# NSAPH-Projects/weather2alert

Hardware: AMD Instinct MI355X
Metric: env_steps_per_sec (higher is better)
Workload: dtype f32 tables, fp64 logit accumulation, f32 sigmoid/reward

## Files before the change

### include/w2a.h

```cpp
#ifndef W2A_H
#define W2A_H

#include <stddef.h>
#include <stdint.h>

#ifdef __cplusplus
extern "C" {
#endif

#define W2A_ABI_VERSION 18
#define W2A_ROW_FLOATS 32

enum {
  W2A_OK = 0,
  W2A_ERR_ARG = -1,
  W2A_ERR_SCHEMA = -2,
  W2A_ERR_HIP = -3,
  W2A_ERR_STATE = -4
};

enum {
  W2A_ST_BAD_EPISODE = 1,
  W2A_ST_BAD_ACTION = 2,
  W2A_ST_STEP_AFTER_DONE = 4,
  W2A_ST_STALE_GRAPH = 8
};

enum { W2A_ACT_I32 = 0, W2A_ACT_I64 = 1, W2A_ACT_U8 = 2 };

enum {
  W2A_STEP_AUTORESET = 1,
  W2A_STEP_NO_OBS = 2,
  W2A_STEP_CLASSIC = 8,
  W2A_STEP_WIDE = 32,
  W2A_STEP_UNPACKED = 128,
  W2A_STEP_NEXT_STEP = 256,
  W2A_STEP_NO_CAPTURE = 512,
  W2A_STEP_SKIP_FINISHED = 64,
  W2A_STEP_REWARD_GIVEN = 16
};

enum { W2A_BUDGET_FIXED = 0, W2A_BUDGET_LESS_THAN = 1, W2A_BUDGET_CENTERED = 2 };

typedef struct w2a_tables {
  const float *X;
  const int32_t *n_days;
  const int32_t *B0;
  const float *W;
  const int32_t *fips_to_weather;
  const int32_t *sim_cnt;
  int32_t T, S_w, Y, S, n_samples;
  int32_t n_obs;
  int32_t obs_slot[W2A_ROW_FLOATS];
  int32_t slot_heat_qi;
  const int32_t *sim_ptr;
  const int32_t *sim_idx;
  int32_t slot_alerts_2wks;
  const uint32_t *gate_bits;
  int32_t gate_words;
} w2a_tables;

typedef struct w2a_env w2a_env;

typedef struct w2a_state_view {
  int32_t *t, *used, *streak, *hist14, *last_actual, *at_budget, *budget, *n_days;
  int32_t *county_w, *year_i, *coef_col, *sample, *sticky_budget, *episode_no;
  int32_t *finished;
  float *episode_return;
} w2a_state_view;

int w2a_abi_version(void);
const char *w2a_last_error(void);

size_t w2a_state_bytes(int64_t num_envs);

int w2a_create(const w2a_tables *tables, int64_t num_envs, int64_t env_gid0, void *state, size_t state_bytes,
               int32_t *status, w2a_env **out);
void w2a_destroy(w2a_env *env);

int w2a_reset(w2a_env *env, const int32_t *county_w, const int32_t *year_i, const int32_t *coef_col,
              const int32_t *sample, const int32_t *budget, const uint8_t *mask, float *obs, void *stream);

int w2a_reset_device_rng(w2a_env *env, uint64_t seed, int32_t location, int augment, int32_t budget_kw,
                         int sample_budget_mode, int sticky, int restart_episodes, const uint8_t *mask, float *obs,
                         void *stream);

int w2a_set_autoreset(w2a_env *env, uint64_t seed, int32_t location, int augment, int32_t budget_kw,
                      int sample_budget_mode, int sticky);

int w2a_step(w2a_env *env, const void *actions, int action_dtype, float *obs, float *reward, uint8_t *done,
// ... 332 lines not shown
```

### weather2alert_amd/_ffi.py

```python
from __future__ import annotations

import ctypes as C
import os

from . import build as _build

ROW_FLOATS = 32

OK = 0
ST_BAD_EPISODE, ST_BAD_ACTION, ST_STEP_AFTER_DONE, ST_STALE_GRAPH = 1, 2, 4, 8
ACT_I32, ACT_I64, ACT_U8 = 0, 1, 2
STEP_AUTORESET, STEP_NO_OBS, STEP_CLASSIC, STEP_REWARD_GIVEN, STEP_WIDE, STEP_SKIP_FINISHED, STEP_UNPACKED, STEP_NEXT_STEP, STEP_NO_CAPTURE = 1, 2, 8, 16, 32, 64, 128, 256, 512
S64_MIN_ENVS = 131072
ABI_VERSION = 18
FIX_BITS = {"alert_2wks": 1, "lag": 2, "penalty": 4, "obs": 8, "augment": 16}
BUDGET_FIXED, BUDGET_LESS_THAN, BUDGET_CENTERED = 0, 1, 2

SYMBOLS = [
    "w2a_abi_version", "w2a_last_error", "w2a_state_bytes", "w2a_create", "w2a_destroy", "w2a_reset",
    "w2a_reset_device_rng", "w2a_set_autoreset", "w2a_step", "w2a_get_state", "w2a_read_status",
    "w2a_sort_workspace_bytes", "w2a_sort_episodes", "w2a_reset_device_rng_sorted", "w2a_observe", "w2a_rollout", "w2a_rollout_order_workspace_bytes", "w2a_rollout_order_attach", "w2a_rollout_order", "w2a_rollout_posterior_mean", "w2a_policy_actions", "w2a_set_semantics",
    "w2a_group_workspace_bytes", "w2a_group_by_column", "w2a_posterior_mean_reward", "w2a_set_posterior_kernel", "w2a_set_episode_word", "w2a_invalidate", "w2a_query", "w2a_rollout_mfma_workspace_bytes", "w2a_rollout_mfma_prepare",
    "w2a_rollout_linear", "w2a_rollout_mlp", "w2a_rollout_linear_record", "w2a_rollout_mlp_record",
    "w2a_posterior_returns", "w2a_hindsight_workspace_bytes", "w2a_hindsight_optimum",
    "w2a_policy_gradient_workspace_bytes", "w2a_policy_gradient_linear",
    "w2a_policy_gradient_mlp_workspace_bytes", "w2a_policy_gradient_mlp",
    "w2a_imitation_gradient_linear", "w2a_imitation_gradient_mlp_workspace_bytes", "w2a_imitation_gradient_mlp",
    "w2a_imitation_gradient_linear_weighted", "w2a_imitation_gradient_mlp_weighted",
    "w2a_value_gradient_linear_workspace_bytes", "w2a_value_gradient_linear",
    "w2a_value_gradient_mlp_workspace_bytes", "w2a_value_gradient_mlp",
    "w2a_value_gradient_linear_gae_workspace_bytes", "w2a_value_gradient_linear_gae",
    "w2a_value_gradient_mlp_gae_workspace_bytes", "w2a_value_gradient_mlp_gae",
    "w2a_surrogate_gradient_linear", "w2a_surrogate_gradient_mlp_workspace_bytes", "w2a_surrogate_gradient_mlp",
    "w2a_alert_gate", "w2a_rollout_linear_gated", "w2a_policy_gradient_linear_gated",
    "w2a_imitation_gradient_linear_gated", "w2a_surrogate_gradient_linear_gated", "w2a_hindsight_optimum_gated",
    "w2a_rollout_mlp_gated", "w2a_policy_gradient_mlp_gated", "w2a_imitation_gradient_mlp_gated",
    "w2a_surrogate_gradient_mlp_gated",
    "w2a_fisher_vector_product_linear", "w2a_fisher_vector_product_mlp_workspace_bytes",
    "w2a_fisher_vector_product_mlp",
    "w2a_q_gradient_mlp_workspace_bytes", "w2a_q_gradient_mlp",
    "w2a_actor_critic_mlp_workspace_bytes", "w2a_actor_critic_mlp",
    "w2a_lookahead_rollout_linear", "w2a_lookahead_rollout_linear_gated", "w2a_lookahead_rollout_mlp",
    "w2a_lookahead_rollout_mlp_gated", "w2a_lookahead_policy_gradient_linear",
    "w2a_lookahead_imitation_gradient_linear",
    "w2a_hindsight_along", "w2a_relabel_imitation_linear", "w2a_relabel_imitation_mlp",
    "w2a_hindsight_curve_workspace_bytes", "w2a_hindsight_curve", "w2a_hindsight_curve_gated",
]
Q_LOCKSTEP_DAY, Q_PACKED_ELIGIBLE, Q_PACKED_CURRENT, Q_CANONICAL_CURRENT, Q_LAST_ROLLOUT_KERNEL, Q_LAST_STEP_KERNEL, Q_LOCKSTEP = 0, 1, 2, 3, 4, 5, 6
Q_EPISODE_WORD_BYTES = 7
ROLLOUT_KERNELS = {0: "k_rollout", 1: "k_rollout64", 2: "k_rollout_mfma", 3: "k_rollout_linear", 4: "k_rollout_mlp"}
PM_KERNELS = {"vector": 0, "matrix": 1, "matrix_i8": 2}
POLICY_KINDS = {"never": 0, "always": 1, "bernoulli": 2, "threshold": 3, "table": 4}


class Policy(C.Structure):
    _fields_ = [("kind", C.c_int32), ("p", C.c_float), ("obs_col", C.c_int32), ("threshold", C.c_float),
                ("obs_lag", C.c_int32), ("require_budget", C.c_int32), ("table", C.c_void_p),
                ("table_R", C.c_int32), ("seed", C.c_uint64)]


class LinearPolicy(C.Structure):
    _fields_ = [("weight", C.c_void_p), ("bias", C.c_void_p), ("group", C.c_void_p), ("n_groups", C.c_int32),
                ("sample", C.c_int32), ("require_budget", C.c_int32), ("seed", C.c_uint64)]


# ... 264 lines not shown
```

### weather2alert_amd/csrc/w2a_bookkeeping.h

```cpp
#ifndef W2A_BOOKKEEPING_H
#define W2A_BOOKKEEPING_H

#include <stdint.h>

struct W2aBook {
  int pk_valid, canon_valid;
  int pk_static_ok;
  int lock;
  int32_t uni_t;
  int32_t uni_nd;
  int graph_canon;
  int graph_packed;
  int graph_autoreset;
  int poisoned;
  int perm_valid;
  int has_order;
  int rm_valid;
  int has_order_ws;
  int hist_valid;
  int last_step_kernel, last_rollout_kernel;
};

enum { W2A_BK_STEP_CLASSIC = 0, W2A_BK_STEP_WIDE = 1, W2A_BK_STEP_PACKED = 2 };
enum { W2A_BK_ROLLOUT_4LANE = 0, W2A_BK_ROLLOUT_WIDE = 1, W2A_BK_ROLLOUT_MFMA = 2 };
// ... 59 lines not shown
  const bool unpacked = (masked || observe_only) && !before.canon_valid;
  b = before;
  if (unpacked) b.canon_valid = 1;
  b.hist_valid = 0; b.perm_valid = 0; b.rm_valid = 0;
}

struct BkStepPlan {
  int kernel;
  int32_t uni_nd;
  int converted;
};
template <class Dev>
static inline BkStepPlan bk_step(W2aBook &b, Dev &d, bool wide_wanted, bool autoreset, bool given, bool unpacked_flag,
                                 bool capturing) {
  BkStepPlan p;
  p.kernel = W2A_BK_STEP_CLASSIC; p.uni_nd = b.uni_nd; p.converted = 0;
  bool packed = wide_wanted && !given && !unpacked_flag && bk_can_pack(b);
  if (capturing) {
    if (packed && !b.pk_valid) packed = false;
    if (!packed && !b.canon_valid) { p.kernel = -1; return p; }
  }
  if (autoreset) {
    b.perm_valid = 0;
    b.rm_valid = 0;
    b.hist_valid = 0;
  }
  if (capturing) {
    if (packed) b.graph_packed = 1;
    else b.graph_canon = 1;
    if (autoreset) b.graph_autoreset = 1;
  }
  int32_t uni_next = (!autoreset && b.uni_t >= 0 && b.uni_t + 1 < b.uni_nd) ? b.uni_t + 1 : -1;
  if (bk_any_graph(b)) uni_next = -1;
  if (packed) {
    if (!b.pk_valid) {
      d.pack_state();
      b.pk_valid = 1; b.poisoned = 0;
      p.converted = 1;
    }
    p.kernel = W2A_BK_STEP_PACKED;
    b.canon_valid = 0;
    b.uni_t = uni_next;
    b.last_step_kernel = W2A_BK_STEP_PACKED;
    return p;
  }
  if (wide_wanted) p.kernel = W2A_BK_STEP_WIDE;
  if (!b.canon_valid) p.converted = 2;
  bk_ensure_canonical(b, d);
  bk_canonical_modified(b, true);
  b.uni_t = uni_next;
  b.last_step_kernel = p.kernel;
  return p;
}
static inline void bk_step_rollback(W2aBook &b, const W2aBook &before, const BkStepPlan &p) {
  const W2aBook after = b;
  b = before;
  b.graph_canon = after.graph_canon; b.graph_packed = after.graph_packed; b.graph_autoreset = after.graph_autoreset;
  if (bk_any_graph(b)) b.uni_t = -1;
  if (p.converted == 1) { b.pk_valid = 1; b.poisoned = 0; }
  if (p.converted == 2) b.canon_valid = 1;
}

template <class Dev>
static inline bool bk_rollout_begin(W2aBook &b, Dev &d, int32_t n_steps) {
  const int32_t day = b.uni_t;
  bk_ensure_canonical(b, d);
  bk_canonical_modified(b, true);
  b.uni_t = (day >= 0 && day + n_steps < b.uni_nd && !bk_any_graph(b)) ? day + n_steps : -1;
  return b.lock != 0;
}
static inline int bk_rollout_kernel(W2aBook &b, bool lock, bool fixes, bool mfma_built, bool wide_built) {
  int k = (wide_built && b.has_order) ? W2A_BK_ROLLOUT_WIDE : W2A_BK_ROLLOUT_4LANE;
  if (b.rm_valid && b.has_order && !fixes && lock && mfma_built) k = W2A_BK_ROLLOUT_MFMA;
  b.last_rollout_kernel = k;
  return k;
}

template <class Dev>
static inline void bk_sort(W2aBook &b, Dev &d) {
  bk_ensure_canonical(b, d);
  bk_canonical_modified(b, true);
  b.rm_valid = 0;
  b.perm_valid = 0;
  b.hist_valid = 0;
}
static inline void bk_grouped(W2aBook &b) { b.perm_valid = b.graph_autoreset ? 0 : 1; }
static inline void bk_order_attach(W2aBook &b, bool drops_order = false) {
  b.has_order_ws = 1; b.hist_valid = 0;
  if (drops_order) { b.has_order = 0; b.rm_valid = 0; }
}
static inline void bk_order_set(W2aBook &b) { b.has_order = 1; b.rm_valid = 0; }
static inline void bk_rm_prepared(W2aBook &b) { b.rm_valid = b.graph_autoreset ? 0 : 1; }

static inline void bk_invalidate(W2aBook &b) {
  b.pk_valid = 0; b.canon_valid = 1; b.lock = 0; b.uni_t = -1; b.perm_valid = 0;
  b.rm_valid = 0;
  b.hist_valid = 0;
  b.poisoned = 0;
}

#endif
```

### weather2alert_amd/csrc/w2a_step64.hip.h

```cpp
#ifndef W2A_STEP64_HIP_H
#define W2A_STEP64_HIP_H

#ifndef W2A_S64_MIN_ENVS
#define W2A_S64_MIN_ENVS 131072
#endif
#define S64_ENVS 64
#define S64_WAVES (BLOCK / 64)
#define S64_PASS_ENVS 32
#define S64_ROUNDS 4
#define S64_LIST_ROUNDS 4

struct Day {
  uint32_t t, used, streak, hist, ndays, atb, actual, used2, hist2, st_bits, last;
  int32_t budget, act;
  bool done;
};
__device__ __forceinline__ Day derive_day(const u3 h, const u3 c, int32_t act) {
  Day d;
  d.st_bits = 0;
  if (act != 0 && act != 1) { d.st_bits |= W2A_ST_BAD_ACTION; act = 1; }
  d.act = act;
  d.last = D0_LAST(h.a);
  d.t = D0_T(h.a); d.used = D0_USED(h.a); d.streak = D0_STREAK(h.a);
  d.hist = D1_HIST(h.b); d.ndays = D1_NDAYS(h.b);
// ... 63 lines not shown
#ifndef W2A_S64_SERPENTINE
#define W2A_S64_SERPENTINE 1
#endif
__device__ __forceinline__ uint32_t logical_block_rev(uint32_t b, uint32_t per_xcd) {
#if W2A_XCD_SWIZZLE
  return (b & 7u) * per_xcd + (per_xcd - 1u - (b >> 3));
#else
  return 8u * per_xcd - 1u - b;
#endif
}
template <bool WRITE_OBS, bool REWARD_GIVEN, bool AUTORESET, bool FIXES>
__host__ __device__ constexpr int s64_issue_rounds() {
  return (!WRITE_OBS || (FIXES && !AUTORESET)) ? S64_ROUNDS : 2 * S64_ROUNDS;
}
template <bool WRITE_OBS, bool REWARD_GIVEN, bool PACKED, bool AUTORESET = false, bool FIXES = false, bool NARROW = false>
__device__ __forceinline__ void s64_tile(const StepArgs &a, S64WaveT<FIXES> &sw, const int lane, const int64_t wave_env0,
                                         const bool valid, const uint32_t e, const u3 h, const u3 c, const int32_t act,
                                         const int4 so) {
  const Day d = derive_day(h, c, act);
  const uint32_t t = d.t, used2 = d.used2, hist2 = d.hist2, streak = d.streak, ndays = d.ndays;
  const uint32_t actual = d.actual, atb = d.atb, st_bits = d.st_bits;
  const int32_t budget = d.budget;
  const bool done = d.done;
  const bool restart_in = AUTORESET && a.next_step && D1_FIN(h.b);
  const uint32_t pk0 = NARROW ? pk_rem8(budget - (int32_t)used2) : used2;
  if (NARROW && (uint32_t)budget >= PK_REM_ESCAPE && valid && !restart_in && !(a.skip_finished && D1_FIN(h.b)))
    pk_rem_of(a.st, a.n)[e] = (uint32_t)(budget - (int32_t)used2);
  const uint32_t fx = FIXES ? a.tb.fixes : 0u;
  const bool fix_obs = FIXES && WRITE_OBS && (fx & W2A_FIX_OBS);
  uint32_t need_eff = actual;
  if (a.tb.gate_bits && actual)
    need_eff = (a.tb.gate_bits[t * (uint32_t)a.tb.gate_words + (c.b >> 5)] >> (c.b & 31u)) & 1u;
  const unsigned long long eff_mask = REWARD_GIVEN ? 0ull : __ballot(need_eff != 0u);
  const int n_eff = __popcll(eff_mask);
  if (!REWARD_GIVEN && need_eff)
    sw.elist[__builtin_amdgcn_mbcnt_hi((uint32_t)(eff_mask >> 32), __builtin_amdgcn_mbcnt_lo((uint32_t)eff_mask, 0u))] = (uint8_t)lane;
  {
    const uint32_t day_row = t * (uint32_t)(a.tb.S_w * a.tb.Y) + c.b;
    const uint32_t wrow = NARROW ? c.c : W_COL(c.c) * (uint32_t)a.tb.n_samples + W_SAMPLE(c.c);
    sw.desc[lane] = make_uint2((day_row * (ROWF / 4)) | ((fix_obs && !done) ? 0x80000000u : 0u),
                               (wrow * (2 * ROWF / 4)) | (need_eff << 31));
    sw.rt[lane] = runtime_fields(d, (fx & W2A_FIX_LAG) != 0u);
    if (fix_obs)
      sw.rt2[FIXES ? lane : 0] = make_float4((float)actual, (float)(actual ? streak + 1 : 0), (float)(budget - (int32_t)used2),
                                 (float)__popc(hist2));
  }
  __builtin_amdgcn_fence(__ATOMIC_RELEASE, "wavefront");
  __builtin_amdgcn_wave_barrier();
  __builtin_amdgcn_fence(__ATOMIC_ACQUIRE, "wavefront");

  const int p = lane & 7;
  const int g = lane >> 3;
  const int n_obs = a.tb.n_obs;
  const bool write_me = valid && (!done || fix_obs) && !restart_in;
  const uint32_t next_day = (uint32_t)(a.tb.S_w * a.tb.Y) * (ROWF / 4);
  constexpr int NI = s64_issue_rounds<WRITE_OBS, REWARD_GIVEN, AUTORESET, FIXES>();
  auto eff_issue = [&](const int idx, float4 &xe, float4 &we, int &je) {
    const bool has = idx < n_eff;
    je = has ? (int)sw.elist[idx & (S64_ENVS - 1)] : g;
    const uint2 ds = sw.desc[je];
    xe = a.tb.X[(ds.x & 0x7FFFFFFFu) + p];
    we = a.tb.W[(ds.y & 0x7FFFFFFFu) + (has ? ROWF / 4 : 0) + p];
  };
  auto eff_logit = [&](const int idx, float4 xe, const float4 we, const int je) {
    if (p == RT_QUAD) xe = sw.rt[je];
    if (FIXES && (fx & W2A_FIX_ALERTS_2WKS) && a.tb.slot_hist2w >= 0 && p == (a.tb.slot_hist2w >> 2))
      set_comp4(xe, a.tb.slot_hist2w & 3, sw.rt[je].w);
    double ze = (double)xe.x * (double)we.x;
    ze = fma((double)xe.y, (double)we.y, ze);
    ze = fma((double)xe.z, (double)we.z, ze);
    ze = fma((double)xe.w, (double)we.w, ze);
    if (p == GATE_QUAD && !(xe.z > 0.5f)) ze = -__builtin_inf();
    ze += dpp_f64<0xB1>(ze);
    ze += dpp_f64<0x4E>(ze);
    ze += dpp_f64<0x141>(ze);
    if (p == 0 && idx < n_eff) sw.z[je].y = (float)ze;
  };
  float4 lx0 = make_float4(0.f, 0.f, 0.f, 0.f), lw0 = lx0;
  int lj0 = 0;
  if (!REWARD_GIVEN && NI < 2 * S64_ROUNDS) eff_issue(g, lx0, lw0, lj0);
#pragma unroll 1
  for (int r0 = 0; r0 < S64_ENVS / 8; r0 += NI) {
    if (REWARD_GIVEN && !WRITE_OBS) break;
    if (wave_env0 + r0 * 8 >= a.n) break;
    float4 x[NI], wb[NI], xo[FIXES ? NI : 1];
    bool nxt[NI];
#pragma unroll
    for (int r = 0; r < NI; ++r) {
      uint2 ds = sw.desc[(r0 + r) * 8 + g];
      nxt[r] = FIXES && (ds.x >> 31) != 0u;
      if (FIXES) ds.x &= 0x7FFFFFFFu;
      x[r] = a.tb.X[ds.x + p];
      if (fix_obs) xo[r] = a.tb.X[ds.x + (nxt[r] ? next_day : 0u) + p];
      wb[r] = make_float4(0.f, 0.f, 0.f, 0.f);
      if (!REWARD_GIVEN) wb[r] = a.tb.W[(ds.y & 0x7FFFFFFFu) + p];
      if (!REWARD_GIVEN && NI == 2 * S64_ROUNDS && r == S64_ROUNDS - 1) eff_issue(g, lx0, lw0, lj0);
    }
#if W2A_S64_PRIO
    __builtin_amdgcn_s_setprio(W2A_S64_PRIO);
#endif
#pragma unroll
    for (int r = 0; r < NI; ++r) {
      const int j = (r0 + r) * 8 + g;
      if (p == RT_QUAD) x[r] = sw.rt[j];
      if (FIXES && (fx & W2A_FIX_ALERTS_2WKS) && a.tb.slot_hist2w >= 0) {
        const float a2w = sw.rt[j].w;
        if (p == (a.tb.slot_hist2w >> 2)) set_comp4(x[r], a.tb.slot_hist2w & 3, a2w);
// ... 102 lines not shown
    const float eff = need_eff ? sigmoid_f32(z.y) : 0.0f;
    r = -(1000.0f / 152.0f) * base * (1.0f - eff);
    if (FIXES && (fx & W2A_FIX_PENALTY) && d.act == 1 && atb) r = -1.0f;
  }
  const uint32_t t2 = done ? t : t + 1;
  const uint32_t streak2 = done ? streak : (actual ? streak + 1 : 0);
  const float ret = __uint_as_float(h.c) + r;
  u3 h2;
  h2.a = pack_d0(t2, used2, streak2, actual, atb);
  h2.b = pack_d1(hist2, ndays, done ? 1u : 0u);
  h2.c = __float_as_uint(ret);
#if W2A_S64_SC1 & 2
  if (PACKED) st8_sc1(&a.st.pk_hot[e], v2u{pk_pack_hot(pk0, streak2, hist2, done ? 1u : 0u), h2.c});
  else st12_sc1(&a.st.hot3[e], v3u{h2.a, h2.b, h2.c});
  if (!REWARD_GIVEN) st4_sc1(&a.reward[e], __float_as_uint(r));
  st1_sc1(&a.done[e], done ? 1u : 0u);
#else
  if (PACKED) a.st.pk_hot[e] = make_uint2(pk_pack_hot(pk0, streak2, hist2, done ? 1u : 0u), h2.c);
  else a.st.hot3[e] = h2;
  if (!REWARD_GIVEN) a.reward[e] = r;
  a.done[e] = done ? 1 : 0;
#endif
  if (PACKED && lane == 0) a.st.pk_day[wave_env0 >> 6] = t2;
  if (done && a.last_return) a.last_return[e] = ret;
  if (st_bits) atomicOr(a.status, (int)st_bits);
  }
  if (AUTORESET) {
    const bool rs = valid && (a.next_step ? restart_in : done);
    const unsigned long long rs_mask = __ballot(rs);
    if (rs_mask) {
      uint2 ds = make_uint2(0xFFFFFFFFu, 0u);
      if (rs) {
        const uint4 cold = load_cold(a.st, e);
        const Episode ep = draw_episode(a.tb, a.rc, (uint64_t)(a.gid0 + e), cold.w + 1, (int32_t)cold.z);
        if (ep.bad) atomicOr(a.status, (int)W2A_ST_BAD_EPISODE);
        store_episode(a.st, e, make_uint4(ep.ep_row, ep.ep_w, (uint32_t)ep.sticky, cold.w + 1),
                      make_uint4(pack_d0(0, 0, 0, 0, 0), pack_d1(0, ep.ndays, 0), __float_as_uint(0.0f), (uint32_t)ep.budget));
        if (PACKED && NARROW) {
          a.st.pk_hot[e] = make_uint2(pk_pack_hot(pk_rem8(ep.budget), 0u, 0u, 0u), __float_as_uint(0.0f));
          reinterpret_cast<uint32_t *>(a.st.pk_c)[e] = pk_narrow_word(ep.ep_row, ep.ep_w, (uint32_t)a.tb.n_samples, a.pk_kw);
          pk_rem_of(a.st, a.n)[e] = (uint32_t)ep.budget;
        } else if (PACKED) {
          a.st.pk_hot[e] = make_uint2(pk_pack_hot(0u, 0u, 0u, 0u), __float_as_uint(0.0f));
          a.st.pk_c[e] = make_uint2(pk_budget16((uint32_t)ep.budget) | (W_COL(ep.ep_w) << 16),
                                    (ep.ep_row & 0x3FFFFFu) | (W_SAMPLE(ep.ep_w) << 22));
        }
        ds = make_uint2(ep.ep_row * (ROWF / 4), (uint32_t)ep.budget);
      }
      if (WRITE_OBS) {
        sw.desc[lane] = ds;
        __builtin_amdgcn_fence(__ATOMIC_RELEASE, "wavefront");
        __builtin_amdgcn_wave_barrier();
        __builtin_amdgcn_fence(__ATOMIC_ACQUIRE, "wavefront");
#pragma unroll 1
        for (int r = 0; r < S64_ENVS / 8; ++r) {
          if (!((rs_mask >> (r * 8)) & 0xFFull)) continue;
          const int j = r * 8 + g;
          const uint2 dj = sw.desc[j];
          if (dj.x != 0xFFFFFFFFu) {
            float4 v = a.tb.X[dj.x + p];
            if (p == RT_QUAD) v = make_float4(0.0f, 0.0f, (float)(int32_t)dj.y, 0.0f);
            if (FIXES && (fx & W2A_FIX_ALERTS_2WKS) && a.tb.slot_hist2w >= 0 && p == (a.tb.slot_hist2w >> 2))
              set_comp4(v, a.tb.slot_hist2w & 3, 0.0f);
            float *row = reinterpret_cast<float *>(a.obs) + (size_t)(wave_env0 + j) * n_obs;
            if (so.x >= 0) row[so.x] = v.x;
            if (so.y >= 0) row[so.y] = v.y;
            if (so.z >= 0) row[so.z] = v.z;
            if (so.w >= 0) row[so.w] = v.w;
          }
        }
      }
      if (PACKED && lane == 0) a.st.pk_day[wave_env0 >> 6] = 0u;
    }
  }
}

template <bool NARROW>
__device__ __forceinline__ void s64_load_packed(const StepArgs &a, uint32_t e, uint32_t day, u3 &h, u3 &c, int32_t &act) {
  if (NARROW) {
    const uint32_t *ew = reinterpret_cast<const uint32_t *>(a.st.pk_c);
#if W2A_S64_NT_STATE & 4
    const v2u phv = __builtin_nontemporal_load(reinterpret_cast<const v2u *>(&a.st.pk_hot[e]));
    const uint2 ph = make_uint2(phv.x, phv.y);
    const uint32_t w = __builtin_nontemporal_load(&ew[e]);
#else
    const uint2 ph = a.st.pk_hot[e];
    const uint32_t w = ew[e];
#endif
    const uint32_t used = 0u;
    c.a = PK_USED(ph.x);
    if (c.a == PK_REM_ESCAPE) c.a = pk_rem_of(a.st, a.n)[e];
    h.a = pack_d0(day, used, PK_STREAK(ph.x), PK_HIST(ph.x) & 1u, 0u);
    h.b = pack_d1(PK_HIST(ph.x), (uint32_t)a.uni_nd, PK_FIN(ph.x));
    h.c = ph.y;
    c.b = w >> a.pk_kw;
    c.c = w & ((1u << a.pk_kw) - 1u);
    act = load_action(a, e);
    return;
  }
#if W2A_S64_NT_STATE & 4
  const v2u phv = __builtin_nontemporal_load(reinterpret_cast<const v2u *>(&a.st.pk_hot[e]));
  const v2u pcv = __builtin_nontemporal_load(reinterpret_cast<const v2u *>(&a.st.pk_c[e]));
  const uint2 ph = make_uint2(phv.x, phv.y), pc = make_uint2(pcv.x, pcv.y);
#else
  const uint2 ph = a.st.pk_hot[e];
  const uint2 pc = a.st.pk_c[e];
#endif
  h.a = pack_d0(day, PK_USED(ph.x), PK_STREAK(ph.x), PK_HIST(ph.x) & 1u, 0u);
  h.b = pack_d1(PK_HIST(ph.x), (uint32_t)a.uni_nd, PK_FIN(ph.x));
  h.c = ph.y;
  c.a = pc.x & 0xFFFFu;
  if (c.a == PK_BUDGET_ESCAPE) c.a = a.st.stepc[e].a;
  c.b = pc.y & 0x3FFFFFu;
  c.c = PACK_W(pc.x >> 16, pc.y >> 22);
  act = load_action(a, e);
}
__device__ __forceinline__ void s64_load_state(const StepArgs &a, uint32_t e, u3 &h, u3 &c, int32_t &act) {
#if W2A_S64_NT_STATE & 1
  const v3u hv = __builtin_nontemporal_load(reinterpret_cast<const v3u *>(&a.st.hot3[e]));
  h.a = hv.x; h.b = hv.y; h.c = hv.z;
#else
// ... 106 lines not shown
```

### weather2alert_amd/csrc/w2a_step_dispatch.hip.h

```cpp
#ifndef W2A_STEP_DISPATCH_HIP_H
#define W2A_STEP_DISPATCH_HIP_H

int w2a_step(w2a_env *env, const void *actions, int action_dtype, float *obs, float *reward, uint8_t *done,
             float *last_return, int flags, void *stream) {
  if (!env || !actions || !reward || !done) return fail(W2A_ERR_ARG, "w2a_step: NULL argument");
  if (action_dtype < W2A_ACT_I32 || action_dtype > W2A_ACT_U8) return fail(W2A_ERR_ARG, "w2a_step: bad action_dtype");
  const bool no_obs = (flags & W2A_STEP_NO_OBS) != 0;
  const bool autoreset = (flags & W2A_STEP_AUTORESET) != 0;
  const bool given = (flags & W2A_STEP_REWARD_GIVEN) != 0;
  if (given && (autoreset || env->tb.fixes || (flags & W2A_STEP_CLASSIC)))
    return fail(W2A_ERR_ARG, "w2a_step: W2A_STEP_REWARD_GIVEN is served by the 64-envs-per-wave kernel only (no in-kernel "
                             "autoreset, no corrected-semantics flags)");
  if (!no_obs && !obs) return fail(W2A_ERR_ARG, "w2a_step: obs is NULL (pass W2A_STEP_NO_OBS for reward-only)");
  if (!no_obs && ((uintptr_t)obs & 15)) return fail(W2A_ERR_ARG, "w2a_step: obs must be 16-B aligned");
  if (autoreset && !env->has_autoreset) return fail(W2A_ERR_ARG, "w2a_step: W2A_STEP_AUTORESET needs w2a_set_autoreset first");
  StepArgs a;
  memset(&a, 0, sizeof(a));
  a.tb = env->tb; a.slot_obs = env->slot_obs; a.st = env->st;
  a.actions = actions; a.obs = obs; a.reward = reward; a.done = done; a.last_return = last_return;
  a.status = env->status; a.n = env->n; a.gid0 = env->gid0; a.rc = env->autoreset; a.act_dtype = action_dtype;
  a.skip_finished = (flags & W2A_STEP_SKIP_FINISHED) ? 1 : 0;
  a.next_step = (flags & W2A_STEP_NEXT_STEP) ? 1 : 0;
  if (a.next_step && !autoreset) return fail(W2A_ERR_ARG, "w2a_step: W2A_STEP_NEXT_STEP goes with W2A_STEP_AUTORESET");
  if (a.skip_finished && !given)
    return fail(W2A_ERR_ARG, "w2a_step: W2A_STEP_SKIP_FINISHED goes with W2A_STEP_REWARD_GIVEN (policy loops)");
  dim3 grid(grid_for(env->n)), block(BLOCK);
  hipStream_t s = (hipStream_t)stream;
  const bool capturing = stream_is_capturing(s);
  if (capturing && (flags & W2A_STEP_NO_CAPTURE))
    return fail(W2A_ERR_STATE, "w2a_step: the stream is recording a hipGraph, but this loop's episode boundaries are driven "
                               "from the host (W2A_STEP_NO_CAPTURE): a reset between two steps cannot be recorded. Let the "
                               "step kernel restart finished envs itself (W2A_STEP_AUTORESET; HeatAlertVecEnv(lockstep=False))");
  const bool wide = (given || (flags & W2A_STEP_WIDE) || env->n >= W2A_S64_MIN_ENVS) && !(flags & W2A_STEP_CLASSIC);
  HipDev dv{env, s};
  const W2aBook before = env->bk;
  const BkStepPlan plan = bk_step(env->bk, dv, wide, autoreset, given, (flags & W2A_STEP_UNPACKED) != 0, capturing);
  if (plan.kernel < 0)
    return fail(W2A_ERR_STATE, "w2a_step: this step runs on the canonical state words, which are not current (the state is "
                               "in its packed lock-step form), and a conversion cannot be recorded into a hipGraph; call "
                               "w2a_get_state before capturing -- or, on a handle with a recorded packed step, do not "
                               "record a step of another kind");
#define W2A_STEP_TRY(expr) \
  do { hipError_t _e = (expr); \
       if (_e != hipSuccess) { bk_step_rollback(env->bk, before, plan); if (!capturing) bk_end_call(env->bk, dv); \
                               return fail(W2A_ERR_HIP, #expr ": %s", hipGetErrorString(_e)); } } while (0)
  if (plan.kernel != W2A_BK_STEP_CLASSIC) {
    const int64_t per_wg = (int64_t)BLOCK * W2A_S64_TILES;
    const int64_t tiles = (env->n + per_wg - 1) / per_wg;
    dim3 grid64((unsigned)(((tiles + 7) / 8) * 8));
    a.walk_rev = env->s64_launches++ & 1u;
    a.pk_kw = -1;
    if (plan.kernel == W2A_BK_STEP_PACKED) {
      a.uni_nd = plan.uni_nd;
      a.pk_kw = env->ew.narrow ? env->ew.kw : -1;
#define W2A_LAUNCH_PK(NW)                                                                                                \
      do {                                                                                                               \
        if (autoreset) {   \
          if (env->tb.fixes) {                                                                                           \
            if (no_obs) hipLaunchKernelGGL((k_step64<false, false, true, true, true, NW>), grid64, block, 0, s, a);      \
            else hipLaunchKernelGGL((k_step64<true, false, true, true, true, NW>), grid64, block, 0, s, a);              \
          } else if (no_obs) hipLaunchKernelGGL((k_step64<false, false, true, true, false, NW>), grid64, block, 0, s, a); \
          else hipLaunchKernelGGL((k_step64<true, false, true, true, false, NW>), grid64, block, 0, s, a);               \
        } else if (env->tb.fixes) {   \
          if (no_obs) hipLaunchKernelGGL((k_step64<false, false, true, false, true, NW>), grid64, block, 0, s, a);       \
          else hipLaunchKernelGGL((k_step64<true, false, true, false, true, NW>), grid64, block, 0, s, a);               \
        } else if (no_obs) hipLaunchKernelGGL((k_step64<false, false, true, false, false, NW>), grid64, block, 0, s, a); \
        else hipLaunchKernelGGL((k_step64<true, false, true, false, false, NW>), grid64, block, 0, s, a);                \
      } while (0)
      if (env->ew.narrow) W2A_LAUNCH_PK(true);
      else W2A_LAUNCH_PK(false);
#undef W2A_LAUNCH_PK
      W2A_STEP_TRY(hipGetLastError());
      bk_end_call(env->bk, dv);
      return W2A_OK;
    }
    if (given) {
      if (no_obs) hipLaunchKernelGGL((k_step64<false, true>), grid64, block, 0, s, a);
      else hipLaunchKernelGGL((k_step64<true, true>), grid64, block, 0, s, a);
    } else if (env->tb.fixes) {
      if (autoreset) {
        if (no_obs) hipLaunchKernelGGL((k_step64<false, false, false, true, true>), grid64, block, 0, s, a);
        else hipLaunchKernelGGL((k_step64<true, false, false, true, true>), grid64, block, 0, s, a);
      } else {
        if (no_obs) hipLaunchKernelGGL((k_step64<false, false, false, false, true>), grid64, block, 0, s, a);
        else hipLaunchKernelGGL((k_step64<true, false, false, false, true>), grid64, block, 0, s, a);
      }
    } else if (autoreset) {
      if (no_obs) hipLaunchKernelGGL((k_step64<false, false, false, true>), grid64, block, 0, s, a);
      else hipLaunchKernelGGL((k_step64<true, false, false, true>), grid64, block, 0, s, a);
    } else {
      if (no_obs) hipLaunchKernelGGL((k_step64<false, false>), grid64, block, 0, s, a);
      else hipLaunchKernelGGL((k_step64<true, false>), grid64, block, 0, s, a);
    }
    W2A_STEP_TRY(hipGetLastError());
    if (!capturing) bk_end_call(env->bk, dv);
    return W2A_OK;
  }
#define W2A_LAUNCH(AR, OB) \
  do { if (env->tb.fixes) hipLaunchKernelGGL((k_step<AR, OB, true>), grid, block, 0, s, a); \
       else hipLaunchKernelGGL((k_step<AR, OB, false>), grid, block, 0, s, a); } while (0)
  if (autoreset) { if (no_obs) W2A_LAUNCH(true, false); else W2A_LAUNCH(true, true); }
  else { if (no_obs) W2A_LAUNCH(false, false); else W2A_LAUNCH(false, true); }
#undef W2A_LAUNCH
  W2A_STEP_TRY(hipGetLastError());
#undef W2A_STEP_TRY
  if (!capturing) bk_end_call(env->bk, dv);
  return W2A_OK;
}

#endif
```

### weather2alert_amd/env.py

```python
from __future__ import annotations

import ctypes as C
from typing import Literal

import numpy as np
import torch

from . import _ffi, policy as _policy, stats as _stats
from .info import _LazyInfo
from .options import KernelOptions
from .rng import numpy_parity_episode
from .spaces import Box, Discrete
from .tables import CompiledTables, DeviceTables, compile_from_files

_ACT_CODES = {torch.int32: _ffi.ACT_I32, torch.int64: _ffi.ACT_I64, torch.uint8: _ffi.ACT_U8,
              torch.bool: _ffi.ACT_U8}
_BUDGET_MODES = {"less_than": _ffi.BUDGET_LESS_THAN, "centered": _ffi.BUDGET_CENTERED}
_cur_device = getattr(torch._C, "_cuda_getDevice", torch.cuda.current_device)

try:
    from gymnasium.vector import VectorEnv as _VectorEnvBase
except ImportError:
    _VectorEnvBase = object
try:
# ... 159 lines not shown
                self._group_ws = torch.empty(self._lib.w2a_group_workspace_bytes(n, ct.S, ct.n_samples), dtype=torch.uint8,
                                             device=dev)
        nd = np.unique(ct.n_days)
        uniform = len(nd) == 1 and nd[0] > 0
        if episode_order == "sorted":
            if not uniform:
                raise ValueError("episode_order='sorted' needs one episode length for every (county, year)")
            if lockstep is False:
                raise ValueError("episode_order='sorted' implies lockstep")
            with torch.cuda.device(dev):
                self._sort_ws = torch.empty(self._lib.w2a_sort_workspace_bytes(n), dtype=torch.uint8, device=dev)
        if lockstep and not uniform:
            raise ValueError("lockstep=True needs one episode length for every (county, year)")
        self._episode_len = int(nd[0]) if uniform else 0
        self._lockstep = bool(uniform and self.seed_mode == "device" and lockstep is not False)
        self._steps_in_episode = 0
        self._pending_reset = False
        self._reset_cfg = None
        self._set_step_mode()
        self._w2a_step = self._lib.w2a_step
        self._raw_stream = getattr(torch._C, "_cuda_getCurrentRawStream", None)
        self._sticky = [budget] * n
        self._needs_reset = True
        self._obs_current = False
        self._last_opts: dict = {}
        self._np_random = None
        self._np_random_seed = None

    @property
    def unwrapped(self):
        return self

    @property
    def np_random(self) -> np.random.Generator:
        if self._np_random is None:
            self._np_random_seed = int(np.random.SeedSequence().entropy % (2**63))
            self._np_random = np.random.default_rng(self._np_random_seed)
        return self._np_random

    @np_random.setter
    def np_random(self, value: np.random.Generator):
        self._np_random, self._np_random_seed = value, -1

    @property
    def np_random_seed(self):
        self.np_random
        return self._np_random_seed

    def _set_step_mode(self):
        auto = self.autoreset in ("same_step", "next_step") and self.seed_mode == "device"
        self._dev_auto = auto and not self._lockstep
        self._host_auto = auto and self._lockstep and self.autoreset == "same_step"
        self._host_next = auto and self._lockstep and self.autoreset == "next_step"
        if not self._host_next:
            self._pending_reset = False
        if self.reward_mode == "posterior_mean" and self._dev_auto:
            raise ValueError("reward_mode='posterior_mean' cannot run with the in-kernel autoreset (batches that left "
                             "lock step); use autoreset='disabled' or whole-batch resets")
        self._pm = self.reward_mode == "posterior_mean"
        host_driven = self._host_auto or self._host_next or (self.autoreset == "same_step" and not self._dev_auto)
        self._step_flags = ((0 if self.write_obs else _ffi.STEP_NO_OBS) |
                            (_ffi.STEP_NO_CAPTURE if host_driven else 0) |
                            (_ffi.STEP_REWARD_GIVEN if self._pm else 0) |
                            (_ffi.STEP_CLASSIC if self.step_kernel == "classic" else 0) |
                            (_ffi.STEP_WIDE if self.step_kernel in ("wide", "wide_unpacked") else 0) |
                            (_ffi.STEP_UNPACKED if self.step_kernel in ("unpacked", "wide_unpacked") else 0) |
                            (_ffi.STEP_AUTORESET if self._dev_auto else 0) |
                            (_ffi.STEP_NEXT_STEP if self._dev_auto and self.autoreset == "next_step" else 0))

    @property
    def step_kernel_name(self) -> str:
        wide = self._pm or self.step_kernel in ("wide", "wide_unpacked") or (self.step_kernel in ("auto", "unpacked") and
                                                          self.num_envs >= _ffi.S64_MIN_ENVS)
        return "k_step64" if (wide and self.step_kernel != "classic") else "k_step"

    @property
    def last_step_kernel(self) -> str | None:
        return {0: "k_step", 1: "k_step64", 2: "k_step64<packed>"}.get(
            self._lib.w2a_query(self._h, _ffi.Q_LAST_STEP_KERNEL))

    @property
    def packed_state(self) -> bool:
        return bool(self._lib.w2a_query(self._h, _ffi.Q_PACKED_CURRENT)) and not bool(
            self._lib.w2a_query(self._h, _ffi.Q_CANONICAL_CURRENT))

    @property
    def episode_word_bytes(self) -> int:
        return int(self._lib.w2a_query(self._h, _ffi.Q_EPISODE_WORD_BYTES))

    @property
    def last_rollout_kernel(self) -> str | None:
        return _ffi.ROLLOUT_KERNELS.get(self._lib.w2a_query(self._h, _ffi.Q_LAST_ROLLOUT_KERNEL))

    def _stream(self):
        if self._raw_stream is not None:
            return self._raw_stream(self._dev_index)
        return torch.cuda.current_stream(self.device).cuda_stream

    def close(self, **kwargs):
        if getattr(self, "_h", None):
            torch.cuda.synchronize(self.device)
            self._lib.w2a_destroy(self._h)
            self._h = None
        self._look_tables = {}
        self.closed = True

# ... 269 lines not shown
            if self.pm_kernel_choice is None:
                self._pick_pm_kernel()

    def _pick_pm_kernel(self, reps: int = 3):
        act = torch.zeros(self.num_envs, dtype=torch.int32, device=self.device)
        best = {}
        with torch.cuda.device(self.device):
            for name, code in _ffi.PM_KERNELS.items():
                _ffi.check(self._lib.w2a_set_posterior_kernel(self._h, code), "w2a_set_posterior_kernel")
                times = []
                for _ in range(reps + 1):
                    e0, e1 = torch.cuda.Event(enable_timing=True), torch.cuda.Event(enable_timing=True)
                    e0.record()
                    _ffi.check(self._lib.w2a_posterior_mean_reward(self._h, act.data_ptr(), _ffi.ACT_I32, self._rew_ptr,
                                                                   self._stream()), "w2a_posterior_mean_reward")
                    e1.record()
                    e1.synchronize()
                    times.append(e0.elapsed_time(e1) * 1e3)
                best[name] = min(times[1:])
            self.pm_kernel_timing_us = best
            self.pm_kernel_choice = min(best, key=best.get)
            if self.pm_sync_group is not None:
                import torch.distributed as td

                names = list(_ffi.PM_KERNELS)
                pick = torch.tensor([names.index(self.pm_kernel_choice)], dtype=torch.int32, device=self.device)
                group = None if self.pm_sync_group is True else self.pm_sync_group
                td.broadcast(pick, src=td.get_global_rank(group, 0) if group is not None else 0, group=group)
                self.pm_kernel_choice = names[int(pick.item())]
            _ffi.check(self._lib.w2a_set_posterior_kernel(self._h, _ffi.PM_KERNELS[self.pm_kernel_choice]),
                       "w2a_set_posterior_kernel")
            self.check_status()

    def step(self, actions):
        if self._needs_reset:
            raise RuntimeError("call reset() before step()")
        if (type(actions) is not torch.Tensor or actions.device != self.device or actions.dtype not in _ACT_CODES
                or actions.numel() != self.num_envs or not actions.is_contiguous()):
            actions = self._coerce_actions(actions)
        if _cur_device() != self._dev_index:
            with torch.cuda.device(self.device):
                return self.step(actions)
        if self._pending_reset:
            self._launch_device_reset(None, self._obs_ptr)
            self._reward.zero_()
            self._done.zero_()
            self._keep_act = actions
            return self._obs, self._reward, self._done_bool, self._truncated, _LazyInfo(self)
        if self._pm:
            rc = self._lib.w2a_posterior_mean_reward(self._h, actions.data_ptr(), _ACT_CODES[actions.dtype],
                                                     self._rew_ptr, self._stream())
            if rc != 0:
                _ffi.check(rc, "w2a_posterior_mean_reward")
        rc = self._w2a_step(self._h, actions.data_ptr(), _ACT_CODES[actions.dtype], self._obs_ptr, self._rew_ptr,
                            self._done_ptr, self._fr_ptr, self._step_flags, self._stream())
        if rc != 0:
            _ffi.check(rc, "w2a_step")
        self._keep_act = actions
        self._obs_current = self.write_obs
        done = self._done_bool
        if self._host_auto:
            self._steps_in_episode += 1
            if self._steps_in_episode == self._episode_len:
                self._launch_device_reset(None, self._obs_ptr)
        elif self._host_next:
            self._steps_in_episode += 1
            if self._steps_in_episode == self._episode_len:
                self._pending_reset = True
        elif self.autoreset == "same_step" and not self._dev_auto:
            d = done.cpu().numpy()
            if d.any():
                self._reset_numpy_parity(None, self._last_opts, d, torch.as_tensor(d.astype(np.uint8),
                                         device=self.device), self._obs_ptr)
        return self._obs, self._reward, done, self._truncated, _LazyInfo(self)

    def record_steps(self, one_day, days: int, warmup: bool = True):
        from .graph import RecordedSteps

        return RecordedSteps(self, one_day, days, warmup)

    def rollout(self, policy: dict, n_steps: int | None = None, alert_mask: bool = False, record: bool = False,
                posterior_returns: bool = False, hindsight: bool = False,
                policy_gradient: bool | str = False) -> dict:
        pg = _policy.check_policy_gradient(policy_gradient, policy.get("kind"), policy.get("sample", False),
                                           self.reward_mode, self.fixes, record, kinds=("linear", "mlp"))
        if self._needs_reset:
            raise RuntimeError("call reset() before rollout()")
        ct = self.ct
        kind = policy.get("kind")
        lin = None
        gate = _policy.check_allowed_days(policy, self.num_envs, ct.T, self.device, "rollout()")
        if record and kind not in ("linear", "mlp"):
            raise ValueError(f"rollout(record=True) needs kind 'linear' or 'mlp', got {kind!r}")
        if posterior_returns and self.fixes - {"budget"}:
            raise ValueError(f"rollout(posterior_returns=True) needs faithful semantics; fixes "
                             f"{sorted(self.fixes - {'budget'})} make the reward depend on attempts and other rows")
        if hindsight:
            self._check_hindsight("rollout(hindsight=True)")
        if kind in ("linear", "mlp"):
            if self._pm:
                raise ValueError(f"rollout(kind={kind!r}) needs reward_mode='sampled'")
            if self.fixes - {"budget"}:
                raise ValueError(f"rollout(kind={kind!r}) needs faithful observations; fixes {sorted(self.fixes - {'budget'})} "
                                 "change what the observation is")
            if policy.get("lookahead") is not None:
                if record:
                    raise ValueError("rollout(record=True) does not take a 'lookahead' policy: the recorded rows would "
                                     "lack the lookahead inputs (a later addition)")
                if pg is not None and kind == "mlp":
                    raise ValueError("rollout(policy_gradient=...) takes 'lookahead' with kind 'linear' only; the mlp "
                                     "kind's gradient kernels do not read the lookahead inputs yet")
            lin = _check_learned(self, policy)
        elif kind not in _ffi.POLICY_KINDS:
            raise ValueError(f"policy kind {kind!r}")
        if self._pending_reset:
            self._launch_device_reset(None, self._obs_ptr)
        if lin is not None and not self._obs_current:
# ... 1031 lines not shown
```

### weather2alert_amd/options.py

```python
from __future__ import annotations

from dataclasses import dataclass, fields, replace
from typing import Literal


@dataclass(frozen=True)
class KernelOptions:
    step_kernel: Literal["auto", "classic", "wide", "unpacked", "wide_unpacked"] = "auto"
    write_obs: bool = True
    reward_path: Literal["gather", "auto", "table"] = "gather"
    rollout_order: bool = True
    rollout_mfma: bool = True
    pm_kernel: Literal["auto", "vector", "matrix", "matrix_i8"] = "matrix_i8"
    sorted_reset: Literal["fused", "relabel"] = "fused"
    force_wide_episode_word: bool = False

    def __post_init__(self):
        if self.step_kernel not in ("auto", "classic", "wide", "unpacked", "wide_unpacked"):
            raise ValueError(f"step_kernel {self.step_kernel!r}")
        if self.reward_path == "table":
            raise ValueError("reward_path='table' (the precomputed logit table of round 1) was removed: it was slower "
                             "than the row-gather kernels at every batch size; use 'gather'")
        if self.reward_path not in ("gather", "auto"):
            raise ValueError(f"reward_path {self.reward_path!r}")
        if self.pm_kernel not in ("auto", "vector", "matrix", "matrix_i8"):
            raise ValueError(f"pm_kernel {self.pm_kernel!r}")
        if self.sorted_reset not in ("fused", "relabel"):
            raise ValueError(f"sorted_reset {self.sorted_reset!r}")

    @classmethod
    def names(cls) -> tuple:
        return tuple(f.name for f in fields(cls))

    def with_overrides(self, **kw) -> "KernelOptions":
        unknown = set(kw) - set(self.names())
        if unknown:
            raise TypeError(f"unexpected keyword argument(s) {sorted(unknown)}")
        return replace(self, **kw) if kw else self
```

Baseline: 32.18 billion.

## Fuse lockstep episode-boundary reset into the final packed step kernel

```diff
diff --git a/include/w2a.h b/include/w2a.h
--- a/include/w2a.h
+++ b/include/w2a.h
@@ -16,7 +16,8 @@
   W2A_ERR_ARG = -1,
   W2A_ERR_SCHEMA = -2,
   W2A_ERR_HIP = -3,
-  W2A_ERR_STATE = -4
+  W2A_ERR_STATE = -4,
+  W2A_DECLINED = 1
 };
 
 enum {
@@ -36,6 +37,7 @@
   W2A_STEP_UNPACKED = 128,
   W2A_STEP_NEXT_STEP = 256,
   W2A_STEP_NO_CAPTURE = 512,
+  W2A_STEP_LOCKSTEP_RESTART = 1024,
   W2A_STEP_SKIP_FINISHED = 64,
   W2A_STEP_REWARD_GIVEN = 16
 };
diff --git a/weather2alert_amd/_ffi.py b/weather2alert_amd/_ffi.py
--- a/weather2alert_amd/_ffi.py
+++ b/weather2alert_amd/_ffi.py
@@ -8,9 +8,11 @@
 ROW_FLOATS = 32
 
 OK = 0
+DECLINED = 1
 ST_BAD_EPISODE, ST_BAD_ACTION, ST_STEP_AFTER_DONE, ST_STALE_GRAPH = 1, 2, 4, 8
 ACT_I32, ACT_I64, ACT_U8 = 0, 1, 2
 STEP_AUTORESET, STEP_NO_OBS, STEP_CLASSIC, STEP_REWARD_GIVEN, STEP_WIDE, STEP_SKIP_FINISHED, STEP_UNPACKED, STEP_NEXT_STEP, STEP_NO_CAPTURE = 1, 2, 8, 16, 32, 64, 128, 256, 512
+STEP_LOCKSTEP_RESTART = 1024
 S64_MIN_ENVS = 131072
 ABI_VERSION = 18
 FIX_BITS = {"alert_2wks": 1, "lag": 2, "penalty": 4, "obs": 8, "augment": 16}
diff --git a/weather2alert_amd/csrc/w2a_bookkeeping.h b/weather2alert_amd/csrc/w2a_bookkeeping.h
--- a/weather2alert_amd/csrc/w2a_bookkeeping.h
+++ b/weather2alert_amd/csrc/w2a_bookkeeping.h
@@ -135,6 +135,14 @@
   b.last_step_kernel = p.kernel;
   return p;
 }
+static inline bool bk_restart_grantable(const W2aBook &b) {
+  return bk_can_pack(b) && !bk_any_graph(b) && b.uni_t >= 0 && b.uni_t + 1 == b.uni_nd;
+}
+static inline void bk_restart_done(W2aBook &b) {
+  if (!b.lock || bk_any_graph(b)) return;
+  b.uni_t = 0;
+  b.canon_valid = 1;
+}
 static inline void bk_step_rollback(W2aBook &b, const W2aBook &before, const BkStepPlan &p) {
   const W2aBook after = b;
   b = before;
diff --git a/weather2alert_amd/csrc/w2a_step64.hip.h b/weather2alert_amd/csrc/w2a_step64.hip.h
--- a/weather2alert_amd/csrc/w2a_step64.hip.h
+++ b/weather2alert_amd/csrc/w2a_step64.hip.h
@@ -139,7 +139,7 @@
   const int p = lane & 7;
   const int g = lane >> 3;
   const int n_obs = a.tb.n_obs;
-  const bool write_me = valid && (!done || fix_obs) && !restart_in;
+  const bool write_me = valid && (!done || (fix_obs && !(AUTORESET && !a.next_step))) && !restart_in;
   const uint32_t next_day = (uint32_t)(a.tb.S_w * a.tb.Y) * (ROWF / 4);
   constexpr int NI = s64_issue_rounds<WRITE_OBS, REWARD_GIVEN, AUTORESET, FIXES>();
   auto eff_issue = [&](const int idx, float4 &xe, float4 &we, int &je) {
@@ -348,21 +348,89 @@
         __builtin_amdgcn_fence(__ATOMIC_RELEASE, "wavefront");
         __builtin_amdgcn_wave_barrier();
         __builtin_amdgcn_fence(__ATOMIC_ACQUIRE, "wavefront");
+        const uint32_t rs_lo = (uint32_t)rs_mask, rs_hi = (uint32_t)(rs_mask >> 32);
+        const bool fast_lo = rs_lo == 0xFFFFFFFFu && wave_env0 + S64_PASS_ENVS <= a.n;
+        const bool fast_hi = rs_hi == 0xFFFFFFFFu && wave_env0 + 2 * S64_PASS_ENVS <= a.n;
+        auto row0 = [&](const int j, float4 &v, uint32_t &bud) {
+          const uint2 dj = sw.desc[j];
+          v = a.tb.X[dj.x + p];
+          bud = dj.y;
+        };
+        auto finish0 = [&](float4 &v, const uint32_t bud) {
+          if (p == RT_QUAD) v = make_float4(0.0f, 0.0f, (float)(int32_t)bud, 0.0f);
+          if (FIXES && (fx & W2A_FIX_ALERTS_2WKS) && a.tb.slot_hist2w >= 0 && p == (a.tb.slot_hist2w >> 2))
+            set_comp4(v, a.tb.slot_hist2w & 3, 0.0f);
+        };
+        auto flush0 = [&](const float4 *v, const int e_off) {
+          const int trash = S64_PASS_ENVS * n_obs + (lane & 31);
+#pragma unroll
+          for (int rr = 0; rr < S64_ROUNDS; ++rr) {
+            const int base = (rr * 8 + g) * n_obs;
+            sw.tile[so.x >= 0 ? base + so.x : trash] = v[rr].x;
+            sw.tile[so.y >= 0 ? base + so.y : trash] = v[rr].y;
+            sw.tile[so.z >= 0 ? base + so.z : trash] = v[rr].z;
+            sw.tile[so.w >= 0 ? base + so.w : trash] = v[rr].w;
+          }
+          __builtin_amdgcn_fence(__ATOMIC_RELEASE, "wavefront");
+          __builtin_amdgcn_wave_barrier();
+          __builtin_amdgcn_fence(__ATOMIC_ACQUIRE, "wavefront");
+          float *dst = reinterpret_cast<float *>(a.obs) + (wave_env0 + e_off) * n_obs;
+          const int chunks = (S64_PASS_ENVS * n_obs) >> 2;
+#pragma unroll
+          for (int c0 = 0; c0 < (S64_PASS_ENVS * ROWF) / 4; c0 += 64) {
+            const int ch = c0 + lane;
+            if (ch < chunks) {
+              const v4f q = reinterpret_cast<const v4f *>(sw.tile)[ch];
+#if W2A_S64_SC1 & 1
+              st16_sc1(reinterpret_cast<v4f *>(dst) + ch, q);
+#elif W2A_NT_OBS
+              __builtin_nontemporal_store(q, reinterpret_cast<v4f *>(dst) + ch);
+#else
+              reinterpret_cast<v4f *>(dst)[ch] = q;
+#endif
+            }
+          }
+          __builtin_amdgcn_fence(__ATOMIC_RELEASE, "wavefront");
+          __builtin_amdgcn_wave_barrier();
+          __builtin_amdgcn_fence(__ATOMIC_ACQUIRE, "wavefront");
+        };
+        if (fast_lo && fast_hi) {
+          float4 v[2 * S64_ROUNDS];
+          uint32_t bud[2 * S64_ROUNDS];
+#pragma unroll
+          for (int r = 0; r < 2 * S64_ROUNDS; ++r) row0(r * 8 + g, v[r], bud[r]);
+#pragma unroll
+          for (int r = 0; r < 2 * S64_ROUNDS; ++r) finish0(v[r], bud[r]);
+          flush0(v, 0);
+          flush0(v + S64_ROUNDS, S64_PASS_ENVS);
+        } else {
 #pragma unroll 1
-        for (int r = 0; r < S64_ENVS / 8; ++r) {
-          if (!((rs_mask >> (r * 8)) & 0xFFull)) continue;
-          const int j = r * 8 + g;
-          const uint2 dj = sw.desc[j];
-          if (dj.x != 0xFFFFFFFFu) {
-            float4 v = a.tb.X[dj.x + p];
-            if (p == RT_QUAD) v = make_float4(0.0f, 0.0f, (float)(int32_t)dj.y, 0.0f);
-            if (FIXES && (fx & W2A_FIX_ALERTS_2WKS) && a.tb.slot_hist2w >= 0 && p == (a.tb.slot_hist2w >> 2))
-              set_comp4(v, a.tb.slot_hist2w & 3, 0.0f);
-            float *row = reinterpret_cast<float *>(a.obs) + (size_t)(wave_env0 + j) * n_obs;
-            if (so.x >= 0) row[so.x] = v.x;
-            if (so.y >= 0) row[so.y] = v.y;
-            if (so.z >= 0) row[so.z] = v.z;
-            if (so.w >= 0) row[so.w] = v.w;
+          for (int half = 0; half < 2; ++half) {
+            if (half ? fast_hi : fast_lo) {
+              float4 v[S64_ROUNDS];
+              uint32_t bud[S64_ROUNDS];
+#pragma unroll
+              for (int r = 0; r < S64_ROUNDS; ++r) row0((half * S64_ROUNDS + r) * 8 + g, v[r], bud[r]);
+#pragma unroll
+              for (int r = 0; r < S64_ROUNDS; ++r) finish0(v[r], bud[r]);
+              flush0(v, half * S64_PASS_ENVS);
+              continue;
+            }
+#pragma unroll 1
+            for (int r = half * S64_ROUNDS; r < (half + 1) * S64_ROUNDS; ++r) {
+              if (!((rs_mask >> (r * 8)) & 0xFFull)) continue;
+              const int j = r * 8 + g;
+              const uint2 dj = sw.desc[j];
+              if (dj.x != 0xFFFFFFFFu) {
+                float4 v = a.tb.X[dj.x + p];
+                finish0(v, dj.y);
+                float *row = reinterpret_cast<float *>(a.obs) + (size_t)(wave_env0 + j) * n_obs;
+                if (so.x >= 0) row[so.x] = v.x;
+                if (so.y >= 0) row[so.y] = v.y;
+                if (so.z >= 0) row[so.z] = v.z;
+                if (so.w >= 0) row[so.w] = v.w;
+              }
+            }
           }
         }
       }
diff --git a/weather2alert_amd/csrc/w2a_step_dispatch.hip.h b/weather2alert_amd/csrc/w2a_step_dispatch.hip.h
--- a/weather2alert_amd/csrc/w2a_step_dispatch.hip.h
+++ b/weather2alert_amd/csrc/w2a_step_dispatch.hip.h
@@ -6,7 +6,8 @@
   if (!env || !actions || !reward || !done) return fail(W2A_ERR_ARG, "w2a_step: NULL argument");
   if (action_dtype < W2A_ACT_I32 || action_dtype > W2A_ACT_U8) return fail(W2A_ERR_ARG, "w2a_step: bad action_dtype");
   const bool no_obs = (flags & W2A_STEP_NO_OBS) != 0;
-  const bool autoreset = (flags & W2A_STEP_AUTORESET) != 0;
+  bool autoreset = (flags & W2A_STEP_AUTORESET) != 0;
+  const bool restart_req = (flags & W2A_STEP_LOCKSTEP_RESTART) != 0;
   const bool given = (flags & W2A_STEP_REWARD_GIVEN) != 0;
   if (given && (autoreset || env->tb.fixes || (flags & W2A_STEP_CLASSIC)))
     return fail(W2A_ERR_ARG, "w2a_step: W2A_STEP_REWARD_GIVEN is served by the 64-envs-per-wave kernel only (no in-kernel "
@@ -14,6 +15,9 @@
   if (!no_obs && !obs) return fail(W2A_ERR_ARG, "w2a_step: obs is NULL (pass W2A_STEP_NO_OBS for reward-only)");
   if (!no_obs && ((uintptr_t)obs & 15)) return fail(W2A_ERR_ARG, "w2a_step: obs must be 16-B aligned");
   if (autoreset && !env->has_autoreset) return fail(W2A_ERR_ARG, "w2a_step: W2A_STEP_AUTORESET needs w2a_set_autoreset first");
+  if (restart_req && (flags & (W2A_STEP_AUTORESET | W2A_STEP_NEXT_STEP | W2A_STEP_REWARD_GIVEN | W2A_STEP_CLASSIC | W2A_STEP_UNPACKED)))
+    return fail(W2A_ERR_ARG, "w2a_step: W2A_STEP_LOCKSTEP_RESTART does not go with AUTORESET, NEXT_STEP, REWARD_GIVEN, CLASSIC "
+                             "or UNPACKED");
   StepArgs a;
   memset(&a, 0, sizeof(a));
   a.tb = env->tb; a.slot_obs = env->slot_obs; a.st = env->st;
@@ -32,6 +36,10 @@
                                "from the host (W2A_STEP_NO_CAPTURE): a reset between two steps cannot be recorded. Let the "
                                "step kernel restart finished envs itself (W2A_STEP_AUTORESET; HeatAlertVecEnv(lockstep=False))");
   const bool wide = (given || (flags & W2A_STEP_WIDE) || env->n >= W2A_S64_MIN_ENVS) && !(flags & W2A_STEP_CLASSIC);
+  if (restart_req) {
+    if (!env->has_autoreset || capturing || !wide || !bk_restart_grantable(env->bk)) return W2A_DECLINED;
+    autoreset = true;
+  }
   HipDev dv{env, s};
   const W2aBook before = env->bk;
   const BkStepPlan plan = bk_step(env->bk, dv, wide, autoreset, given, (flags & W2A_STEP_UNPACKED) != 0, capturing);
@@ -71,6 +79,7 @@
       else W2A_LAUNCH_PK(false);
 #undef W2A_LAUNCH_PK
       W2A_STEP_TRY(hipGetLastError());
+      if (restart_req) bk_restart_done(env->bk);
       bk_end_call(env->bk, dv);
       return W2A_OK;
     }
diff --git a/weather2alert_amd/env.py b/weather2alert_amd/env.py
--- a/weather2alert_amd/env.py
+++ b/weather2alert_amd/env.py
@@ -235,6 +235,10 @@
         self._dev_auto = auto and not self._lockstep
         self._host_auto = auto and self._lockstep and self.autoreset == "same_step"
         self._host_next = auto and self._lockstep and self.autoreset == "next_step"
+        self._fused_boundary = (self._host_auto and self.kernel.lockstep_boundary == "fused" and
+                                self.episode_order == "iid" and self.reward_mode != "posterior_mean" and
+                                (self.step_kernel == "wide" or
+                                 (self.step_kernel == "auto" and self.num_envs >= _ffi.S64_MIN_ENVS)))
         if not self._host_next:
             self._pending_reset = False
         if self.reward_mode == "posterior_mean" and self._dev_auto:
@@ -610,17 +614,28 @@
                                                      self._rew_ptr, self._stream())
             if rc != 0:
                 _ffi.check(rc, "w2a_posterior_mean_reward")
+        fused = self._fused_boundary and self._steps_in_episode + 1 == self._episode_len
         rc = self._w2a_step(self._h, actions.data_ptr(), _ACT_CODES[actions.dtype], self._obs_ptr, self._rew_ptr,
-                            self._done_ptr, self._fr_ptr, self._step_flags, self._stream())
+                            self._done_ptr, self._fr_ptr,
+                            self._step_flags | _ffi.STEP_LOCKSTEP_RESTART if fused else self._step_flags, self._stream())
         if rc != 0:
-            _ffi.check(rc, "w2a_step")
+            if rc == _ffi.DECLINED and fused:
+                fused = False
+                rc = self._w2a_step(self._h, actions.data_ptr(), _ACT_CODES[actions.dtype], self._obs_ptr, self._rew_ptr,
+                                    self._done_ptr, self._fr_ptr, self._step_flags, self._stream())
+            if rc != 0:
+                _ffi.check(rc, "w2a_step")
         self._keep_act = actions
         self._obs_current = self.write_obs
         done = self._done_bool
         if self._host_auto:
             self._steps_in_episode += 1
             if self._steps_in_episode == self._episode_len:
-                self._launch_device_reset(None, self._obs_ptr)
+                if fused:
+                    self._steps_in_episode = 0
+                    self._regroup()
+                else:
+                    self._launch_device_reset(None, self._obs_ptr)
         elif self._host_next:
             self._steps_in_episode += 1
             if self._steps_in_episode == self._episode_len:
diff --git a/weather2alert_amd/options.py b/weather2alert_amd/options.py
--- a/weather2alert_amd/options.py
+++ b/weather2alert_amd/options.py
@@ -13,6 +13,7 @@
     rollout_mfma: bool = True
     pm_kernel: Literal["auto", "vector", "matrix", "matrix_i8"] = "matrix_i8"
     sorted_reset: Literal["fused", "relabel"] = "fused"
+    lockstep_boundary: Literal["fused", "host"] = "fused"
     force_wide_episode_word: bool = False
 
     def __post_init__(self):
@@ -27,6 +28,8 @@
             raise ValueError(f"pm_kernel {self.pm_kernel!r}")
         if self.sorted_reset not in ("fused", "relabel"):
             raise ValueError(f"sorted_reset {self.sorted_reset!r}")
+        if self.lockstep_boundary not in ("fused", "host"):
+            raise ValueError(f"lockstep_boundary {self.lockstep_boundary!r}")
 
     @classmethod
     def names(cls) -> tuple:
```

New measurement: 32.24 billion, median of 2. Within noise of the previous version (+0.2%).
